# finsberg/fenicsx-beat

Measured on AMD Instinct MI355X. Metric: node_updates_per_sec, higher is better.
Workload: dtype f64

## Files before the change

fenicsx-beat_amd/csrc/beat_pde_rr.hip:

```cpp
#include "beat_pde_internal.h"

#include <algorithm>
#include <cmath>
#include <cstddef>
#include <cstdlib>

namespace {
using namespace beat_pde_detail;

constexpr int SEG = 62;

struct Coef {
  double c[15];
};

struct RGeom {
  int nx, ny, nz;
  int64_t plane;
  int ry;
  int nsegx, nrb, nchunks, zc;
  int total_waves, total_blocks;
  int z_lo_phys, z_hi_phys;
  int z_lo, z_hi;
  int part_off;
  int ghost_lo_tz, ghost_hi_tz;
  int nrg;
};

enum { RR_PDOT = 0, RR_RUPD = 1, RR_RHS = 2, RR_UDOT = 3, RR_PRUPD = 4 };

struct RArgs {
  const double* x;
  const double* x2;
  double* y;
  double* y2;
  const double* tab;
  const double* tab2;
  const double* dinv;
  Coef ci, ci2;
  double dinv_i;
  double cm, omt_dt, dt;
  const double* w[BEAT_MAX_STIM];
  double amp[BEAT_MAX_STIM];
  int nstim;
  double* partials;
  double* st;
  double* alphas;
  int slot;
  const double* e;
  const double* taba;
  Coef cia;
};

struct RKernArgs {
  RGeom g;
  RArgs a;
  const double* X;
  const double* X2;
  double* Y;
  double* Y2;
};

__device__ __forceinline__ double from_left(double v) {
  const int lo = __builtin_amdgcn_update_dpp(0, __double2loint(v), 0x138, 0xf, 0xf, true);
  const int hi = __builtin_amdgcn_update_dpp(0, __double2hiint(v), 0x138, 0xf, 0xf, true);
  return __hiloint2double(hi, lo);
}
__device__ __forceinline__ double from_right(double v) {
  const int lo = __builtin_amdgcn_update_dpp(0, __double2loint(v), 0x130, 0xf, 0xf, true);
  const int hi = __builtin_amdgcn_update_dpp(0, __double2hiint(v), 0x130, 0xf, 0xf, true);
  return __hiloint2double(hi, lo);
}

#ifndef BEAT_RR_BUF
#define BEAT_RR_BUF 2
#endif
typedef int rr_v2i __attribute__((ext_vector_type(2)));
[[maybe_unused]] constexpr unsigned RR_OOB = 0x80000000u;
#ifndef BEAT_RR_NT
#define BEAT_RR_NT 2
#endif
__device__ __forceinline__ void rr_store(double* p, double v) {
#if BEAT_RR_NT & 2
  __builtin_nontemporal_store(v, p);
#else
  *p = v;
#endif
}
__device__ __forceinline__ double rr_buf_load(const double* base, unsigned bytes, unsigned off) {
  const __amdgpu_buffer_rsrc_t r = __builtin_amdgcn_make_buffer_rsrc((void*)base, 0, (int)bytes, 0x00020000);
  const rr_v2i v = __builtin_amdgcn_raw_buffer_load_b64(r, (int)off, 0, (BEAT_RR_NT & 1) ? 2 : 0);
  return __hiloint2double(v.y, v.x);
}

#ifndef BEAT_RR_ALIGN
#define BEAT_RR_ALIGN 1
#endif
__device__ __forceinline__ double from_left_h(double v, double h, int src_lane) {
  const int lo = __builtin_amdgcn_update_dpp(__builtin_amdgcn_readlane(__double2loint(h), src_lane), __double2loint(v), 0x138, 0xf, 0xf, false);
  const int hi = __builtin_amdgcn_update_dpp(__builtin_amdgcn_readlane(__double2hiint(h), src_lane), __double2hiint(v), 0x138, 0xf, 0xf, false);
  return __hiloint2double(hi, lo);
}
__device__ __forceinline__ double from_right_h(double v, double h, int src_lane) {
  const int lo = __builtin_amdgcn_update_dpp(__builtin_amdgcn_readlane(__double2loint(h), src_lane), __double2loint(v), 0x130, 0xf, 0xf, false);
  const int hi = __builtin_amdgcn_update_dpp(__builtin_amdgcn_readlane(__double2hiint(h), src_lane), __double2hiint(v), 0x130, 0xf, 0xf, false);
  return __hiloint2double(hi, lo);
}
#ifndef BEAT_RR_ALIGN_RHS
#define BEAT_RR_ALIGN_RHS 0
#endif
constexpr bool rr_aligned_mode(int mode) {
  return BEAT_RR_ALIGN == 1 && BEAT_RR_BUF != 0 && (mode == 0 || mode == 1 || mode == 3 || mode == 4 || (mode == 2 && BEAT_RR_ALIGN_RHS == 1));
}

__device__ __forceinline__ int axis_type3(int i, int n, int lo_phys, int hi_phys) {
  if (n == 1 && lo_phys && hi_phys) return 1;
  if (i == 0 && lo_phys) return 0;
  if (i == n - 1 && hi_phys) return 2;
  return 1;
}

__device__ __forceinline__ int xcd_block(int b, int total) {
  const int per = (total + 7) >> 3;
  return (b & 7) * per + (b >> 3);
}

#ifndef BEAT_RR_WAVES_RHS
#define BEAT_RR_WAVES_RHS 3
#endif
#ifndef BEAT_RR_WAVES_IT
#define BEAT_RR_WAVES_IT 1
#endif
template <int MODE, int RY, int PD, bool GUESS = false, bool PRED = false>
__global__ __launch_bounds__(BEAT_BLOCK, (GUESS && RY == 2 && PD == 1) ? BEAT_RR_WAVES_RHS : ((MODE == RR_PDOT || MODE == RR_RUPD) && PD == 1 ? BEAT_RR_WAVES_IT : 1)) void rr_kernel(RGeom g, RArgs a, const double* __restrict__ X,
                                                        const double* __restrict__ X2, double* __restrict__ Y,
                                                        double* __restrict__ Y2) {
  constexpr int NR = RY + 2;
  constexpr int NE = GUESS ? NR : 1;
  constexpr bool FORM = MODE == RR_PDOT || MODE == RR_UDOT || MODE == RR_PRUPD;
  constexpr bool OLD = MODE == RR_PDOT || MODE == RR_PRUPD;
  constexpr bool RAW = MODE == RR_UDOT || MODE == RR_PRUPD;
  constexpr int NW = RAW ? RY : 1;
  constexpr bool BUF = BEAT_RR_BUF == 1 || (BEAT_RR_BUF == 2 && (MODE != RR_RHS || BEAT_RR_ALIGN_RHS == 1));
  constexpr bool ALIGNED = rr_aligned_mode(MODE);
  static_assert(!ALIGNED || BUF, "aligned segments come with the raw-buffer loads");
  constexpr int SEGW = ALIGNED ? 64 : SEG;
  static_assert(!GUESS || MODE == RR_RHS, "the initial guess enters the right-hand side only");
  static_assert(!PRED || MODE == RR_PDOT, "the predicted-stop sums come with PDOT only");
  __shared__ double red[4];
  __shared__ double s_dinv[32];
  __shared__ double s_tab[27 * TABW];
  __shared__ double s_tab2[MODE == RR_RHS ? 27 * TABW : 1];
  __shared__ double s_taba[GUESS ? 27 * TABW : 1];
  __shared__ double s_rc[PRED ? 4 * 2 * RY * 64 : 1];
  __shared__ double s_acc[PRED ? 4 * 2 * 64 : 1];
  if (MODE != RR_RHS) {
    if (a.st[STOP] != 0.0) return;
  }
  if (PRED) s_acc[(threadIdx.x >> 6) * 128 + (threadIdx.x & 63)] = s_acc[(threadIdx.x >> 6) * 128 + 64 + (threadIdx.x & 63)] = 0.0;
  for (int i = threadIdx.x; i < 27 * TABW; i += BEAT_BLOCK) {
    s_tab[i] = a.tab[i];
    if (MODE == RR_RHS) s_tab2[i] = a.tab2[i];
    if (GUESS) s_taba[i] = a.taba[i];
  }
  if (threadIdx.x < 27) s_dinv[threadIdx.x] = a.dinv[threadIdx.x];
  __syncthreads();
  const int lane = threadIdx.x & 63;
  const int blk = xcd_block(blockIdx.x, g.total_blocks);
  const int w = blk * 4 + (threadIdx.x >> 6);
  int seg = w % g.nsegx;
  int rb = (w / g.nsegx) % g.nrb;
  int chunk = w / (g.nsegx * g.nrb);
  bool wave_ok = blk < g.total_blocks && w < g.total_waves;
  if (g.nrg > 0) {
    seg = blk % g.nsegx;
    rb = ((blk / g.nsegx) % g.nrg) * 4 + (int)(threadIdx.x >> 6);
    chunk = blk / (g.nsegx * g.nrg);
    wave_ok = blk < g.total_blocks && rb < g.nrb;
  }
  const int gx = seg * SEGW + (ALIGNED ? 0 : -1) + lane;
  const int y0 = rb * RY - 1;
  const int zb = g.z_lo + chunk * g.zc;
  const int ze = wave_ok ? min(zb + g.zc, g.z_hi) : zb;
  const bool x_in = wave_ok && gx >= 0 && gx < g.nx;
  const bool x_out = x_in && (ALIGNED || (lane >= 1 && lane <= SEG));
  const int tx = axis_type3(gx, g.nx, 1, 1);
  bool row_in[NR];
  int txy[NR];
  int off[NR];
  const int cx = min(max(gx, 0), g.nx - 1);
#pragma unroll
  for (int r = 0; r < NR; ++r) {
    const int gy = y0 + r;
    row_in[r] = x_in && gy >= 0 && gy < g.ny;
    txy[r] = tx + 3 * axis_type3(gy, g.ny, 1, 1);
    off[r] = min(max(gy, 0), g.ny - 1) * g.nx + cx;
    if constexpr (BUF) off[r] = row_in[r] ? (int)((unsigned)(gy * g.nx + gx) * 8u) : (int)RR_OOB;
  }
  [[maybe_unused]] const unsigned pbytes = (unsigned)(g.plane * 8);
  [[maybe_unused]] unsigned hoff = RR_OOB;
  [[maybe_unused]] int htxy = 13 % 9;
  if constexpr (ALIGNED) {
    const int hr = lane < 8 ? lane : lane - 8;
    const int hx = lane < 8 ? seg * SEGW - 1 : seg * SEGW + SEGW;
    const int hy = y0 + hr;
    const bool hv = wave_ok && (lane < NR || (lane >= 8 && lane < 8 + NR)) && hx >= 0 && hx < g.nx && hy >= 0 && hy < g.ny;
    hoff = hv ? (unsigned)(hy * g.nx + hx) * 8u : RR_OOB;
    htxy = axis_type3(min(max(hx, 0), g.nx - 1), g.nx, 1, 1) + 3 * axis_type3(min(max(hy, 0), g.ny - 1), g.ny, 1, 1);
  }
  double beta = 0.0, alpha = 0.0;
  if (OLD) beta = a.st[BETA];
  if (MODE == RR_PRUPD) alpha = a.st[ALPHA];
  if (MODE == RR_RUPD) {
    alpha = a.st[RZ] / a.st[PQ];
    if (blockIdx.x == 0 && threadIdx.x == 0) a.alphas[a.slot] = alpha;
  }
  const bool have_old = beta != 0.0;

  double acc0 = 0.0, acc1 = 0.0, acc2 = 0.0;
  double Cm[NR], C0[NR], Cp[NR], ra[PD][NR], rb2[PD][NR];
  double rvn[PD][RY];
  [[maybe_unused]] double Hm = 0.0, H0 = 0.0, Hp = 0.0, rha[PD], rhb[PD];
  [[maybe_unused]] double HEm = 0.0, HE0 = 0.0, HEp = 0.0;
#pragma unroll
  for (int u = 0; u < PD; ++u) rha[u] = rhb[u] = 0.0;
  double Rw0[NW], Rwp[NW];
#pragma unroll
  for (int j = 0; j < NW; ++j) Rw0[j] = Rwp[j] = 0.0;
  double Em[NE], E0[NE], Ep[NE], re1[PD][NE];
#pragma unroll
  for (int r = 0; r < NE; ++r) {
    Em[r] = E0[r] = Ep[r] = 0.0;
#pragma unroll
    for (int u = 0; u < PD; ++u) re1[u][r] = 0.0;
  }
#pragma unroll
  for (int r = 0; r < NR; ++r) {
    Cm[r] = C0[r] = Cp[r] = 0.0;
#pragma unroll
    for (int u = 0; u < PD; ++u) ra[u][r] = rb2[u][r] = 0.0;
  }
#pragma unroll
  for (int u = 0; u < PD; ++u)
#pragma unroll
    for (int j = 0; j < RY; ++j) rvn[u][j] = 0.0;
  for (int zz = zb - 2 - PD; zz < ze; zz += PD) {
#pragma unroll
  for (int u = 0; u < PD; ++u) {
    const int z = zz + u;
    if (z < ze) {
    const int k = z + 1;
    if (k >= zb - 1 && k <= ze) {
      [[maybe_unused]] const bool zok = (k >= 0 || !g.z_lo_phys) && (k < g.nz || !g.z_hi_phys);
      const int tz9 = 9 * (k < 0 ? g.ghost_lo_tz : k >= g.nz ? g.ghost_hi_tz : axis_type3(k, g.nz, g.z_lo_phys, g.z_hi_phys));
      const bool own_plane = (k >= zb && k < ze) || (k == -1 && zb == 0 && !g.z_lo_phys) ||
                             (k == g.nz && ze == g.nz && !g.z_hi_phys);
#pragma unroll
      for (int r = 0; r < NR; ++r) {
        double c = ra[u][r];
        if (RAW && r >= 1 && r <= RY) Rwp[RAW ? r - 1 : 0] = c;
        if (FORM) {
          const int type = txy[r] + tz9;
          const double di = s_dinv[type];
          c = have_old ? fma(beta, rb2[u][r], di * ra[u][r]) : di * ra[u][r];
        }
        if constexpr (!BUF) c = (zok && row_in[r]) ? c : 0.0;
        Cp[r] = c;
        if (GUESS) {
          constexpr int q = GUESS ? 1 : 0;
          if constexpr (BUF)
            Ep[r * q] = c + re1[u][r * q];
          else
            Ep[r * q] = (zok && row_in[r]) ? c + re1[u][r * q] : 0.0;
        }
        if (OLD) {
          if (own_plane && r >= 1 && r <= RY && x_out && row_in[r])
            rr_store(&Y[(int64_t)k * g.plane + (int64_t)(y0 + r) * g.nx + gx], c);
        }
        if (PRED && r >= 1 && r <= RY) s_rc[((((threadIdx.x >> 6) * 2 + (k & 1)) * RY) + r - 1) * 64 + lane] = ra[u][r];
      }
      if constexpr (ALIGNED) {
        double hc = rha[u];
        if (FORM) {
          const double di = s_dinv[htxy + tz9];
          hc = have_old ? fma(beta, rhb[u], di * rha[u]) : di * rha[u];
        }
        Hp = hc;
        if (GUESS) HEp = hc + rhb[u];
      }
    }
    double rv[RY];
    if (MODE == RR_RUPD) {
#pragma unroll
      for (int j = 0; j < RY; ++j) rv[j] = rvn[u][j];
      if (z + PD >= zb && z + PD < ze) {
        const double* __restrict__ br = X2 + (int64_t)(z + PD) * g.plane;
#pragma unroll
        for (int j = 0; j < RY; ++j) rvn[u][j] = BUF ? rr_buf_load(br, pbytes, (unsigned)off[j + 1]) : br[off[j + 1]];
      }
    }
    {
      const int kf = k + PD;
      if (kf >= zb - 1 && kf <= ze) {
        const int cz = min(max(kf, -1), g.nz);
        const double* __restrict__ bx = X + (int64_t)cz * g.plane;
        const double* __restrict__ bx2 = (OLD && have_old) ? X2 + (int64_t)cz * g.plane : bx;
        if constexpr (BUF) {
          const unsigned pb = ((kf >= 0 || !g.z_lo_phys) && (kf < g.nz || !g.z_hi_phys)) ? pbytes : 0u;
#pragma unroll
          for (int r = 0; r < NR; ++r) {
            ra[u][r] = rr_buf_load(bx, pb, (unsigned)off[r]);
            if (OLD) rb2[u][r] = rr_buf_load(bx2, pb, (unsigned)off[r]);
          }
          if constexpr (ALIGNED) {
            rha[u] = rr_buf_load(bx, pb, hoff);
            if (OLD) rhb[u] = rr_buf_load(bx2, pb, hoff);
            if (GUESS) rhb[u] = rr_buf_load(X2 + (int64_t)cz * g.plane, pb, hoff);
          }
          if (GUESS) {
            const double* __restrict__ b1 = X2 + (int64_t)cz * g.plane;
#pragma unroll
            for (int r = 0; r < NR; ++r) re1[u][r < NE ? r : 0] = rr_buf_load(b1, pb, (unsigned)off[r]);
          }
        } else {
#pragma unroll
          for (int r = 0; r < NR; ++r) {
            ra[u][r] = bx[off[r]];
            if (OLD) rb2[u][r] = bx2[off[r]];
          }
          if (GUESS) {
            const double* __restrict__ b1 = X2 + (int64_t)cz * g.plane;
#pragma unroll
            for (int r = 0; r < NR; ++r) re1[u][r < NE ? r : 0] = b1[off[r]];
          }
        }
      }
    }
    if (z >= zb) {
    typedef const __attribute__((address_space(4))) char* KArgPtr;
    KArgPtr ka = (KArgPtr)__builtin_amdgcn_kernarg_segment_ptr();
    asm volatile("" : "+s"(ka));
    const RArgs& az = MODE == RR_RHS ? *(const RArgs*)(ka + offsetof(RKernArgs, a)) : a;
    double L0[NR], R0[NR], Rp[NR], Lm[NR];
#pragma unroll
    for (int r = 0; r < NR - 1; ++r) {
      L0[r] = ALIGNED ? from_left_h(C0[r], H0, r) : from_left(C0[r]);
      Lm[r] = ALIGNED ? from_left_h(Cm[r], Hm, r) : from_left(Cm[r]);
    }
#pragma unroll
    for (int r = 1; r < NR; ++r) {
      R0[r] = ALIGNED ? from_right_h(C0[r], H0, 8 + r) : from_right(C0[r]);
      Rp[r] = ALIGNED ? from_right_h(Cp[r], Hp, 8 + r) : from_right(Cp[r]);
    }
    double eL0[NE], eR0[NE], eRp[NE], eLm[NE];
    if (GUESS) {
#pragma unroll
      for (int r = 0; r < NE - 1; ++r) {
        eL0[r] = ALIGNED ? from_left_h(E0[r], HE0, r) : from_left(E0[r]);
        eLm[r] = ALIGNED ? from_left_h(Em[r], HEm, r) : from_left(Em[r]);
      }
#pragma unroll
      for (int r = 1; r < NE; ++r) {
        eR0[r] = ALIGNED ? from_right_h(E0[r], HE0, 8 + r) : from_right(E0[r]);
        eRp[r] = ALIGNED ? from_right_h(Ep[r], HEp, 8 + r) : from_right(Ep[r]);
      }
    }
    const int tz = axis_type3(z, g.nz, g.z_lo_phys, g.z_hi_phys);
#pragma unroll
    for (int j = 0; j < RY; ++j) {
      const int r = j + 1;
      double v[15];
      v[0] = C0[r];
      v[1] = R0[r];
      v[2] = L0[r];
      v[3] = C0[r + 1];
      v[4] = C0[r - 1];
      v[5] = Cp[r];
      v[6] = Cm[r];
      v[7] = R0[r + 1];
      v[8] = L0[r - 1];
      v[9] = Cp[r + 1];
      v[10] = Cm[r - 1];
      v[11] = Rp[r];
      v[12] = Lm[r];
      v[13] = Rp[r + 1];
      v[14] = Lm[r - 1];
      if (x_out && row_in[r]) {
        const int type = txy[r] + 9 * tz;
        const int64_t gi = (int64_t)z * g.plane + (int64_t)(y0 + r) * g.nx + gx;
        double s = 0.0;
#pragma unroll
        for (int k = 0; k < 15; ++k) s = fma(az.ci.c[k], v[k], s);
        if (MODE == RR_RHS) {
          double s2 = 0.0;
          if (!GUESS) {
#pragma unroll
            for (int k = 0; k < 15; ++k) s2 = fma(az.ci2.c[k], v[k], s2);
          }
          double di = s_dinv[13];
          if (type != 13) {
            s = 0.0;
            s2 = 0.0;
#pragma unroll
            for (int k = 0; k < 15; ++k) {
              s = fma(s_tab[type * TABW + k], v[k], s);
              if (!GUESS) s2 = fma(s_tab2[type * TABW + k], v[k], s2);
            }
            di = s_dinv[type];
          }
          double stim = 0.0;
          for (int k = 0; k < az.nstim; ++k) stim = fma(az.amp[k], az.w[k][gi], stim);
          const double b = GUESS ? fma(az.dt, stim, s) : az.cm * s - az.omt_dt * s2 + az.dt * stim;
          double rr = GUESS ? b : az.dt * (stim - s2);
          if (GUESS) {
            constexpr int q = GUESS ? 1 : 0;
            const int re_ = r * q, rp = (r + 1) * q, rm = (r - 1) * q;
            double ev[15];
            ev[0] = E0[re_];
            ev[1] = eR0[re_];
            ev[2] = eL0[re_];
            ev[3] = E0[rp];
            ev[4] = E0[rm];
            ev[5] = Ep[re_];
            ev[6] = Em[re_];
            ev[7] = eR0[rp];
            ev[8] = eL0[rm];
            ev[9] = Ep[rp];
            ev[10] = Em[rm];
            ev[11] = eRp[re_];
            ev[12] = eLm[re_];
            ev[13] = eRp[rp];
            ev[14] = eLm[rm];
            double se = 0.0;
            if (type != 13) {
#pragma unroll
              for (int k = 0; k < 15; ++k) se = fma(s_taba[type * TABW + k], ev[k], se);
            } else {
#pragma unroll
              for (int k = 0; k < 15; ++k) se = fma(az.cia.c[k], ev[k], se);
            }
            rr -= se;
          }
          const double zz = di * rr;
          rr_store(&Y[gi], rr);
          if (Y2 != nullptr) Y2[gi] = v[0];
          acc0 = fma(b, b, acc0);
          acc1 = fma(rr, zz, acc1);
          acc2 = fma(rr, rr, acc2);
        } else {
          double di = s_dinv[13];
          if (type != 13) {
            s = 0.0;
#pragma unroll
            for (int k = 0; k < 15; ++k) s = fma(s_tab[type * TABW + k], v[k], s);
            di = s_dinv[type];
          }
          if (MODE == RR_PDOT) {
            acc0 = fma(v[0], s, acc0);
            if (PRED) {
              double* sa = &s_acc[(threadIdx.x >> 6) * 128 + lane];
              sa[0] = fma(s_rc[((((threadIdx.x >> 6) * 2 + (z & 1)) * RY) + j) * 64 + lane], s, sa[0]);
              sa[64] = fma(s, s, sa[64]);
            }
          } else if (MODE == RR_UDOT) {
            const double ri = Rw0[RAW ? j : 0];
            acc0 = fma(v[0], s, acc0);
            acc1 = fma(ri, v[0], acc1);
            acc2 = fma(ri, ri, acc2);
          } else if (MODE == RR_PRUPD) {
            rr_store(&Y2[gi], fma(-alpha, s, Rw0[RAW ? j : 0]));
          } else {
            const double ri = fma(-alpha, s, rv[j]);
            rr_store(&Y[gi], ri);
            acc0 = fma(ri * di, ri, acc0);
            acc1 = fma(ri, ri, acc1);
          }
        }
      }
    }
    }
#pragma unroll
    for (int r = 0; r < NR; ++r) {
      Cm[r] = C0[r];
      C0[r] = Cp[r];
    }
    if constexpr (ALIGNED) {
      Hm = H0;
      H0 = Hp;
      if (GUESS) {
        HEm = HE0;
        HE0 = HEp;
      }
    }
    if (GUESS) {
#pragma unroll
      for (int r = 0; r < NE; ++r) {
        Em[r] = E0[r];
        E0[r] = Ep[r];
      }
    }
    if (RAW) {
#pragma unroll
      for (int j = 0; j < NW; ++j) Rw0[j] = Rwp[j];
    }
    }
  }
  }

  if (PRED) {
    acc1 = s_acc[(threadIdx.x >> 6) * 128 + (threadIdx.x & 63)];
    acc2 = s_acc[(threadIdx.x >> 6) * 128 + 64 + (threadIdx.x & 63)];
  }
  if (MODE == RR_PDOT && !PRED) {
    const double s0 = beat_block_sum(acc0, red);
    if (threadIdx.x == 0) a.partials[g.part_off + blockIdx.x] = s0;
  } else if (MODE == RR_RUPD) {
    const double s0 = beat_block_sum(acc0, red);
    const double s1 = beat_block_sum(acc1, red);
    if (threadIdx.x == 0) {
      a.partials[g.part_off + blockIdx.x] = s0;
      a.partials[BEAT_MAX_PARTIALS + g.part_off + blockIdx.x] = s1;
    }
  } else if (MODE == RR_PRUPD) {
  } else {
    const double s0 = beat_block_sum(acc0, red);
    const double s1 = beat_block_sum(acc1, red);
    const double s2 = beat_block_sum(acc2, red);
    if (threadIdx.x == 0) {
      a.partials[g.part_off + blockIdx.x] = s0;
      a.partials[BEAT_MAX_PARTIALS + g.part_off + blockIdx.x] = s1;
      a.partials[2 * BEAT_MAX_PARTIALS + g.part_off + blockIdx.x] = s2;
    }
  }
}

__global__ void rr_next_kernel(double* st) {
  if (st[STOP] != 0.0) return;
  st[BETA] = st[RZN] / st[RZ];
  st[RZ] = st[RZN];
  st[RR] = st[RRN];
  st[ITERS] += 1.0;
  const double tr = st[RTOL] * st[RTOL] * st[BB];
  if (st[RR] <= st[TOL2]) {
    st[STOP] = 1.0;
    st[REASON] = st[RR] <= tr ? 2.0 : 3.0;
  } else if (st[ITERS] >= st[MAXIT]) {
    st[STOP] = 1.0;
    st[REASON] = -3.0;
  }
}

__global__ void rr_merged_next_kernel(double* st, double* alphas, int slot) {
  if (st[STOP] != 0.0) return;
  const double g = st[RZN], d = st[PQ], rr = st[RRN];
  st[RR] = rr;
  const double tr = st[RTOL] * st[RTOL] * st[BB];
  if (rr <= st[TOL2]) {
    st[STOP] = 1.0;
    st[REASON] = rr <= tr ? 2.0 : 3.0;
    return;
  }
  if (st[ITERS] >= st[MAXIT]) {
    st[STOP] = 1.0;
    st[REASON] = -3.0;
    return;
  }
  const bool first = st[ITERS] == 0.0;
  const double beta = first ? 0.0 : g / st[RZ];
  const double alpha = first ? g / d : g / (d - beta * g / st[ALPHA]);
  st[BETA] = beta;
  st[ALPHA] = alpha;
  st[RZ] = g;
  alphas[slot] = alpha;
  st[NUPD] += 1.0;
  st[ITERS] += 1.0;
}

int rr_rows(int64_t nodes) {
  static const int forced = [] {
    const char* e = std::getenv("BEAT_RR_RY");
    const int v = e ? std::atoi(e) : 0;
    return (v == 2 || v == 4) ? v : 0;
  }();
  if (forced) return forced;
  return nodes >= ((int64_t)64 << 20) ? 4 : 2;
}

int rr_target_blocks(int64_t nodes) {
  if (const char* e = std::getenv("BEAT_RR_BLOCKS")) return std::max(1, std::atoi(e));
  return nodes >= ((int64_t)64 << 20) ? 4096 : 2048;
}

int rr_prefetch() {
  static const int pd = [] {
    const char* e = std::getenv("BEAT_RR_PD");
    const int v = e ? std::atoi(e) : 1;
    return (v >= 1 && v <= 3) ? v : 1;
  }();
  return pd;
}

int rr_guess_rows() {
  static const int rows = [] {
    const char* e = std::getenv("BEAT_RR_GUESS_RY");
    const int v = e ? std::atoi(e) : 2;
    return v == 4 ? 4 : 2;
  }();
  return rows;
}

int rr_by_rows_mask() {
  static const int mask = [] {
    const char* e = std::getenv("BEAT_RR_BY_ROWS");
    return e ? std::atoi(e) : 0;
  }();
  return mask;
}

RGeom make_geom(const beat_pde* pde, int z_lo, int z_hi, int part_off, int rows = 0, int mode = -1) {
  const Geom& f = pde->g;
  RGeom g{};
  const int64_t nodes = (int64_t)f.nx * f.ny * f.nz;
  const int RY = g.ry = rows ? rows : rr_rows(nodes);
  g.nx = f.nx;
  g.ny = f.ny;
  g.nz = f.nz;
  g.plane = f.plane;
  g.z_lo_phys = f.z_lo_phys;
  g.z_hi_phys = f.z_hi_phys;
  g.z_lo = z_lo;
  g.z_hi = z_hi;
  g.part_off = part_off;
  g.ghost_lo_tz = pde->ghost_lo_tz;
  g.ghost_hi_tz = pde->ghost_hi_tz;
  const int segw = (mode >= 0 && rr_aligned_mode(mode)) ? 64 : SEG;
  g.nsegx = (f.nx + segw - 1) / segw;
  g.nrb = (f.ny + RY - 1) / RY;
  const int nzr = std::max(0, z_hi - z_lo);
  g.nrg = (mode >= 0 && ((rr_by_rows_mask() >> mode) & 1)) ? (g.nrb + 3) / 4 : 0;
  const int64_t per_layer = g.nrg > 0 ? (int64_t)g.nsegx * g.nrg : ((int64_t)g.nsegx * g.nrb + 3) / 4;
  const int target = rr_target_blocks(nodes);
  int nchunks = (int)std::max<int64_t>(1, (target + per_layer - 1) / per_layer);
  nchunks = std::max(1, std::min(nchunks, nzr));
  g.zc = std::max(1, (nzr + nchunks - 1) / nchunks);
  g.nchunks = (nzr + g.zc - 1) / g.zc;
  while ((int64_t)g.nsegx * g.nrb * g.nchunks > (int64_t)2 * BEAT_MAX_PARTIALS && g.nchunks > 1) {
    g.zc *= 2;
    g.nchunks = (nzr + g.zc - 1) / g.zc;
  }
  g.total_waves = g.nsegx * g.nrb * g.nchunks;
  g.total_blocks = (g.total_waves + 3) / 4;
  if (g.nrg > 0) {
    g.total_blocks = g.nsegx * g.nrg * g.nchunks;
    g.total_waves = g.total_blocks * 4;
  }
  return g;
}

RGeom make_geom(const beat_pde* pde) { return make_geom(pde, 0, pde->g.nz, 0); }

inline int grid_blocks(const RGeom& g) { return ((g.total_blocks + 7) / 8) * 8; }
inline int blocks_written(const RGeom& g) { return g.total_blocks > 0 ? grid_blocks(g) : 0; }

Coef interior_row(const double* tab) {
  Coef c;
  for (int k = 0; k < 15; ++k) c.c[k] = tab[13 * 15 + k];
  return c;
}

RArgs rr_operator_args(const beat_pde* pde, double* dev_st) {
  RArgs a{};
  a.tab = pde->d_tab(0);
  a.dinv = pde->d_dinv();
  a.ci = interior_row(pde->h_A);
  a.dinv_i = pde->h_dinv[13];
  a.partials = pde->ctx->d_partials;
  a.st = dev_st;
  return a;
}

template <int MODE, bool GUESS = false, bool PRED = false>
void launch_rr(const beat_pde* pde, const RGeom& g, const RArgs& a) {
  if (g.total_blocks <= 0) return;
  const dim3 grid((unsigned)grid_blocks(g)), block(BEAT_BLOCK);
  hipStream_t s = pde->ctx->stream;
#define BEAT_RR_LAUNCH(RYV, PDV) \
  BEAT_KERNEL((rr_kernel<MODE, RYV, PDV, GUESS, PRED>), grid, block, 0, s, g, a, a.x, GUESS ? a.e : a.x2, a.y, a.y2)
  const int pd = rr_prefetch();
  if (g.ry == 2) {
    if (pd == 2) BEAT_RR_LAUNCH(2, 2); else if (pd == 3) BEAT_RR_LAUNCH(2, 3); else BEAT_RR_LAUNCH(2, 1);
  } else {
    if (pd == 2) BEAT_RR_LAUNCH(4, 2); else if (pd == 3) BEAT_RR_LAUNCH(4, 3); else BEAT_RR_LAUNCH(4, 1);
  }
#undef BEAT_RR_LAUNCH
}
}

bool beat_rr_available(const beat_pde* pde) {
  if (pde->var || pde->pc_ncoef != 1) return false;
  if (const char* e = std::getenv("BEAT_RR")) {
    if (e[0] == '0') return false;
  }
  const RGeom g = make_geom(pde);
  const RGeom gb = make_geom(pde, 0, 1, 0);
  return (int64_t)grid_blocks(g) + 2 * grid_blocks(gb) <= BEAT_MAX_PARTIALS;
}

extern "C" int beat_pde_rr_route(const beat_pde* pde, int* host_out) {
  BEAT_REQUIRE(pde != nullptr && host_out != nullptr, "null argument");
  const RGeom g = make_geom(pde, 0, pde->g.nz, 0, 0, RR_PDOT);
  host_out[0] = beat_rr_available(pde) ? 1 : 0;
  host_out[1] = g.ry;
  host_out[2] = rr_prefetch();
  host_out[3] = rr_by_rows_mask();
  host_out[4] = g.nsegx;
  host_out[5] = g.nrb;
  host_out[6] = g.zc;
  host_out[7] = g.nchunks;
  host_out[8] = g.total_blocks;
  host_out[9] = rr_guess_rows();
  return BEAT_OK;
}

int beat_rr_rhs(beat_pde* pde, const double* dev_v_prev, const double* const* host_dev_stim_w, const double* host_stim_amp,
                int n_stim, double* dev_x, double* dev_r, double* dev_st, int part, const PcgStart* start) {
  BEAT_REQUIRE(start == nullptr || part < 0, "only a right-hand side in one part starts the solve");
  const GuessTerms& gt = pde->guess.cur;
  const bool guess = gt.d != nullptr && gt.use_e;
  const int rows = guess ? rr_guess_rows() : 0;
  RArgs a{};
  a.x = dev_v_prev;
  a.y = dev_r;
  a.y2 = (dev_x == dev_v_prev) ? nullptr : dev_x;
  a.tab = pde->d_tab(2);
  a.tab2 = pde->d_tab(3);
  a.dinv = pde->d_dinv();
  a.ci = interior_row(pde->h_mass);
  a.ci2 = interior_row(pde->h_stiff);
  a.dinv_i = pde->h_dinv[13];
  a.cm = pde->C_m;
  a.omt_dt = (1.0 - pde->theta) * pde->dt;
  a.dt = pde->dt;
  beat_fill_stimuli(a, host_dev_stim_w, host_stim_amp, n_stim);
  a.partials = pde->ctx->d_partials;
  a.st = dev_st;
  if (guess) {
    a.tab = pde->d_tab(1);
    a.ci = interior_row(pde->h_B);
    a.e = gt.e;
    a.taba = pde->d_tab(0);
    a.cia = interior_row(pde->h_A);
  }
  auto launch = [&](int z_lo, int z_hi, int part_off) {
    const RGeom g = make_geom(pde, z_lo, z_hi, part_off, rows, RR_RHS);
    if (guess)
      launch_rr<RR_RHS, true>(pde, g, a);
    else
      launch_rr<RR_RHS>(pde, g, a);
    return blocks_written(g);
  };
  int count = 0;
  if (int rc = beat_launch_parts(pde, PASS_RR_RHS, part, launch, &count)) return rc;
  return part == 0 ? BEAT_OK : beat_pde_launch_reduce(pde, count, 3, dev_st, nullptr, ScalarStep::begin(dev_st, start));
}

double beat_rr_predict_bound(const beat_pde* pde) {
  const Geom& f = pde->g;
  int depth = 0;
  auto chain = [&](const RGeom& g) {
    const int per_thread = (grid_blocks(g) + BEAT_BLOCK - 1) / BEAT_BLOCK;
    depth = std::max(depth, g.zc * g.ry + 8 + per_thread + 8);
  };
  chain(make_geom(pde, 0, f.nz, 0, 0, RR_RHS));
  chain(make_geom(pde, 0, f.nz, 0, 2, RR_RHS));
  chain(make_geom(pde, 0, f.nz, 0, 4, RR_RHS));
  chain(make_geom(pde, 0, f.nz, 0, 0, RR_PDOT));
  chain(make_geom(pde, 0, f.nz, 0, 0, RR_RUPD));
  return 4.0 * (2.0 * depth + 8.0) * std::ldexp(1.0, -53);
}

int beat_rr_pdot_part(beat_pde* pde, double* dev_st, const double* dev_r, const double* dev_p_old, double* dev_p_new,
                      int part, int slot) {
  const Geom& f = pde->g;
  const bool pred = slot >= 0 && pde->predict_stop && f.z_lo_phys && f.z_hi_phys;
  if (pred && pde->predict_c <= 0.0) pde->predict_c = beat_rr_predict_bound(pde);
  RArgs a = rr_operator_args(pde, dev_st);
  a.x = dev_r;
  a.x2 = dev_p_old;
  a.y = dev_p_new;
  auto launch = [&](int z_lo, int z_hi, int part_off) {
    const RGeom g = make_geom(pde, z_lo, z_hi, part_off, 0, RR_PDOT);
    if (pred)
      launch_rr<RR_PDOT, false, true>(pde, g, a);
    else
      launch_rr<RR_PDOT>(pde, g, a);
    return blocks_written(g);
  };
  int count = 0;
  if (int rc = beat_launch_parts(pde, PASS_RR_PDOT, part, launch, &count)) return rc;
  if (part == 0) return BEAT_OK;
  if (pred) {
    static_assert(RQ == PQS + 1 && QQ == PQS + 2, "the three sums are reduced into one run of slots");
    ScalarStep predict{ScalarStep::PREDICT, dev_st};
    predict.alpha_slot = pde->d_alphas + slot;
    predict.bound_c = pde->predict_c;
    return beat_pde_launch_reduce(pde, count, 3, dev_st + PQS, dev_st, predict);
  }
  return beat_pde_launch_reduce(pde, count, 1, dev_st + PQ, dev_st);
}

int beat_rr_pdot(beat_pde* pde, double* dev_st, const double* dev_r, const double* dev_p_old, double* dev_p_new, int slot) {
  if (int rc = beat_rr_pdot_part(pde, dev_st, dev_r, dev_p_old, dev_p_new, 0, slot)) return rc;
  return beat_rr_pdot_part(pde, dev_st, dev_r, dev_p_old, dev_p_new, 1, slot);
}

int beat_rr_rupd(beat_pde* pde, double* dev_st, const double* dev_r, double* dev_r_new, const double* dev_p, int slot,
                 bool roll) {
  const RGeom g = make_geom(pde, 0, pde->g.nz, 0, 0, RR_RUPD);
  RArgs a = rr_operator_args(pde, dev_st);
  a.x = dev_p;
  a.x2 = dev_r;
  a.y = dev_r_new;
  a.alphas = pde->d_alphas;
  a.slot = slot;
  launch_rr<RR_RUPD>(pde, g, a);
  BEAT_LAUNCH_CHECK();
  return beat_pde_launch_reduce(pde, grid_blocks(g), 2, dev_st + RZN, dev_st, ScalarStep::after_update(dev_st, roll));
}

int beat_rr_udot_part(beat_pde* pde, double* dev_st, const double* dev_r, int part) {
  static_assert(RZN == PQ + 1 && RRN == PQ + 2, "the three sums travel as one all-reduce of dev_st[PQ..RRN]");
  RArgs a = rr_operator_args(pde, dev_st);
  a.x = dev_r;
  a.x2 = dev_r;
  auto launch = [&](int z_lo, int z_hi, int part_off) {
    const RGeom g = make_geom(pde, z_lo, z_hi, part_off, 0, RR_UDOT);
    launch_rr<RR_UDOT>(pde, g, a);
    return blocks_written(g);
  };
  int count = 0;
  if (int rc = beat_launch_parts(pde, PASS_RR_UDOT, part, launch, &count)) return rc;
  return part == 0 ? BEAT_OK : beat_pde_launch_reduce(pde, count, 3, dev_st + PQ, dev_st);
}

int beat_rr_merged_next(beat_pde* pde, double* dev_st, int slot) {
  BEAT_KERNEL(rr_merged_next_kernel, dim3(1), dim3(1), 0, pde->ctx->stream, dev_st, pde->d_alphas, slot);
  BEAT_LAUNCH_CHECK();
  return BEAT_OK;
}

int beat_rr_prupd(beat_pde* pde, double* dev_st, const double* dev_r, const double* dev_p_old, double* dev_p_new,
                  double* dev_r_new) {
  const RGeom g = make_geom(pde, 0, pde->g.nz, 0, 0, RR_PRUPD);
  RArgs a = rr_operator_args(pde, dev_st);
  a.x = dev_r;
  a.x2 = dev_p_old;
  a.y = dev_p_new;
  a.y2 = dev_r_new;
  launch_rr<RR_PRUPD>(pde, g, a);
  BEAT_LAUNCH_CHECK();
  return BEAT_OK;
}

int beat_rr_next(beat_pde* pde, double* dev_st) {
  BEAT_KERNEL(rr_next_kernel, dim3(1), dim3(1), 0, pde->ctx->stream, dev_st);
  BEAT_LAUNCH_CHECK();
  return BEAT_OK;
}
```

Baseline: 11.58 billion.

## Pick z-chunk count from kernel occupancy using a wave-fill cost model

Replaces the fixed block target (2048/4096) with a target chosen by minimizing an estimated cost: waves of resident blocks times (chunk depth + prefetch fill), where resident slots come from hipOccupancyMaxActiveBlocksPerMultiprocessor for the exact kernel instantiation. The default row blocking is also changed to 4 rows for all sizes. Large problems still use the old target. The aim is better balance between having enough blocks to fill the GPU and the per-chunk pipeline fill overhead, at the cost of occupancy queries and a small memo per geometry.

Measured after the change: 11.51 billion. No clear change (-0.6%).

```diff
diff --git a/fenicsx-beat_amd/csrc/beat_pde_rr.hip b/fenicsx-beat_amd/csrc/beat_pde_rr.hip
--- a/fenicsx-beat_amd/csrc/beat_pde_rr.hip
+++ b/fenicsx-beat_amd/csrc/beat_pde_rr.hip
@@ -1,8 +1,10 @@
 #include "beat_pde_internal.h"
+#include "beat_rr_fit.h"
 
 #include <algorithm>
 #include <cmath>
 #include <cstddef>
+#include <cstdio>
 #include <cstdlib>
 
 namespace {
@@ -576,20 +578,20 @@
   st[ITERS] += 1.0;
 }
 
-int rr_rows(int64_t nodes) {
+int rr_rows() {
   static const int forced = [] {
     const char* e = std::getenv("BEAT_RR_RY");
     const int v = e ? std::atoi(e) : 0;
     return (v == 2 || v == 4) ? v : 0;
   }();
-  if (forced) return forced;
-  return nodes >= ((int64_t)64 << 20) ? 4 : 2;
-}
-
-int rr_target_blocks(int64_t nodes) {
-  if (const char* e = std::getenv("BEAT_RR_BLOCKS")) return std::max(1, std::atoi(e));
-  return nodes >= ((int64_t)64 << 20) ? 4096 : 2048;
-}
+  return forced ? forced : 4;
+}
+
+constexpr int64_t RR_FIT_BELOW = (int64_t)64 << 20;
+
+constexpr int RR_MAX_BLOCKS = BEAT_MAX_PARTIALS / 2;
+
+int rr_legacy_target(int64_t nodes) { return nodes >= RR_FIT_BELOW ? 4096 : 2048; }
 
 int rr_prefetch() {
   static const int pd = [] {
@@ -600,6 +602,61 @@
   return pd;
 }
 
+template <int MODE, int RY, int PD, bool GUESS, bool PRED>
+int rr_resident_blocks() {
+  static const int slots = [] {
+    int dev = 0, cus = 0, per_cu = 0;
+    if (hipGetDevice(&dev) != hipSuccess || hipDeviceGetAttribute(&cus, hipDeviceAttributeMultiprocessorCount, dev) != hipSuccess ||
+        hipOccupancyMaxActiveBlocksPerMultiprocessor(&per_cu, rr_kernel<MODE, RY, PD, GUESS, PRED>, BEAT_BLOCK, 0) != hipSuccess ||
+        cus < 1 || per_cu < 1) {
+      (void)hipGetLastError();
+      return 0;
+    }
+    if (std::getenv("BEAT_RR_VERBOSE"))
+      std::fprintf(stderr, "rr: mode %d RY %d PD %d guess %d pred %d: %d workgroups per CU x %d CUs\n", MODE, RY, PD, (int)GUESS, (int)PRED, per_cu, cus);
+    return per_cu * cus;
+  }();
+  return slots;
+}
+
+template <int MODE, bool GUESS = false, bool PRED = false>
+int rr_resident_blocks(int ry, int pd) {
+#define BEAT_RR_SLOTS_OF(RYV, PDV) rr_resident_blocks<MODE, RYV, PDV, GUESS, PRED>()
+  if (ry == 2) return pd == 2 ? BEAT_RR_SLOTS_OF(2, 2) : pd == 3 ? BEAT_RR_SLOTS_OF(2, 3) : BEAT_RR_SLOTS_OF(2, 1);
+  return pd == 2 ? BEAT_RR_SLOTS_OF(4, 2) : pd == 3 ? BEAT_RR_SLOTS_OF(4, 3) : BEAT_RR_SLOTS_OF(4, 1);
+#undef BEAT_RR_SLOTS_OF
+}
+
+int rr_slots(int mode, int ry, bool guess, bool pred) {
+  if (const char* e = std::getenv("BEAT_RR_SLOTS")) return std::max(1, std::atoi(e));
+  const int pd = rr_prefetch();
+  switch (mode) {
+    case RR_PDOT: return pred ? rr_resident_blocks<RR_PDOT, false, true>(ry, pd) : rr_resident_blocks<RR_PDOT>(ry, pd);
+    case RR_RUPD: return rr_resident_blocks<RR_RUPD>(ry, pd);
+    case RR_UDOT: return rr_resident_blocks<RR_UDOT>(ry, pd);
+    case RR_PRUPD: return rr_resident_blocks<RR_PRUPD>(ry, pd);
+    default: return guess ? rr_resident_blocks<RR_RHS, true>(ry, pd) : rr_resident_blocks<RR_RHS>(ry, pd);
+  }
+}
+
+int64_t rr_target_blocks(int64_t nodes, int planes, int64_t per_layer, int mode, int ry, bool guess, bool pred) {
+  if (const char* e = std::getenv("BEAT_RR_BLOCKS")) return std::max(1, std::atoi(e));
+  if (nodes >= RR_FIT_BELOW && std::getenv("BEAT_RR_SLOTS") == nullptr) return rr_legacy_target(nodes);
+  const int slots = rr_slots(mode, ry, guess, pred);
+  if (slots <= 0) return rr_legacy_target(nodes);
+  struct Asked {
+    int planes, slots;
+    int64_t per_layer, target;
+  };
+  thread_local Asked memo[8] = {};
+  thread_local int next = 0;
+  for (const Asked& m : memo)
+    if (m.slots == slots && m.planes == planes && m.per_layer == per_layer) return m.target;
+  const int64_t target = rr_fit_target(planes, per_layer, slots, rr_prefetch() + 2, RR_MAX_BLOCKS);
+  memo[next++ & 7] = {planes, slots, per_layer, target};
+  return target;
+}
+
 int rr_guess_rows() {
   static const int rows = [] {
     const char* e = std::getenv("BEAT_RR_GUESS_RY");
@@ -617,11 +674,11 @@
   return mask;
 }
 
-RGeom make_geom(const beat_pde* pde, int z_lo, int z_hi, int part_off, int rows = 0, int mode = -1) {
+RGeom make_geom(const beat_pde* pde, int z_lo, int z_hi, int part_off, int rows = 0, int mode = -1, bool guess = false, bool pred = false) {
   const Geom& f = pde->g;
   RGeom g{};
   const int64_t nodes = (int64_t)f.nx * f.ny * f.nz;
-  const int RY = g.ry = rows ? rows : rr_rows(nodes);
+  const int RY = g.ry = rows ? rows : rr_rows();
   g.nx = f.nx;
   g.ny = f.ny;
   g.nz = f.nz;
@@ -639,15 +696,10 @@
   const int nzr = std::max(0, z_hi - z_lo);
   g.nrg = (mode >= 0 && ((rr_by_rows_mask() >> mode) & 1)) ? (g.nrb + 3) / 4 : 0;
   const int64_t per_layer = g.nrg > 0 ? (int64_t)g.nsegx * g.nrg : ((int64_t)g.nsegx * g.nrb + 3) / 4;
-  const int target = rr_target_blocks(nodes);
-  int nchunks = (int)std::max<int64_t>(1, (target + per_layer - 1) / per_layer);
-  nchunks = std::max(1, std::min(nchunks, nzr));
-  g.zc = std::max(1, (nzr + nchunks - 1) / nchunks);
-  g.nchunks = (nzr + g.zc - 1) / g.zc;
-  while ((int64_t)g.nsegx * g.nrb * g.nchunks > (int64_t)2 * BEAT_MAX_PARTIALS && g.nchunks > 1) {
-    g.zc *= 2;
-    g.nchunks = (nzr + g.zc - 1) / g.zc;
-  }
+  const int64_t target = rr_target_blocks(nodes, nzr, per_layer, mode, RY, guess, pred);
+  const RrChunks cut = rr_chunks(nzr, per_layer, (int64_t)g.nsegx * g.nrb, target, (int64_t)4 * RR_MAX_BLOCKS);
+  g.zc = cut.zc;
+  g.nchunks = cut.nchunks;
   g.total_waves = g.nsegx * g.nrb * g.nchunks;
   g.total_blocks = (g.total_waves + 3) / 4;
   if (g.nrg > 0) {
@@ -752,7 +804,7 @@
     a.cia = interior_row(pde->h_A);
   }
   auto launch = [&](int z_lo, int z_hi, int part_off) {
-    const RGeom g = make_geom(pde, z_lo, z_hi, part_off, rows, RR_RHS);
+    const RGeom g = make_geom(pde, z_lo, z_hi, part_off, rows, RR_RHS, guess);
     if (guess)
       launch_rr<RR_RHS, true>(pde, g, a);
     else
@@ -774,7 +826,10 @@
   chain(make_geom(pde, 0, f.nz, 0, 0, RR_RHS));
   chain(make_geom(pde, 0, f.nz, 0, 2, RR_RHS));
   chain(make_geom(pde, 0, f.nz, 0, 4, RR_RHS));
+  chain(make_geom(pde, 0, f.nz, 0, 2, RR_RHS, true));
+  chain(make_geom(pde, 0, f.nz, 0, 4, RR_RHS, true));
   chain(make_geom(pde, 0, f.nz, 0, 0, RR_PDOT));
+  chain(make_geom(pde, 0, f.nz, 0, 0, RR_PDOT, false, true));
   chain(make_geom(pde, 0, f.nz, 0, 0, RR_RUPD));
   return 4.0 * (2.0 * depth + 8.0) * std::ldexp(1.0, -53);
 }
@@ -789,7 +844,7 @@
   a.x2 = dev_p_old;
   a.y = dev_p_new;
   auto launch = [&](int z_lo, int z_hi, int part_off) {
-    const RGeom g = make_geom(pde, z_lo, z_hi, part_off, 0, RR_PDOT);
+    const RGeom g = make_geom(pde, z_lo, z_hi, part_off, 0, RR_PDOT, false, pred);
     if (pred)
       launch_rr<RR_PDOT, false, true>(pde, g, a);
     else
diff --git a/fenicsx-beat_amd/csrc/beat_rr_fit.h b/fenicsx-beat_amd/csrc/beat_rr_fit.h
--- /dev/null
+++ b/fenicsx-beat_amd/csrc/beat_rr_fit.h
@@ -0,0 +1,52 @@
+#pragma once
+
+#include <algorithm>
+#include <cstdint>
+
+namespace beat_pde_detail {
+
+struct RrChunks {
+  int zc;
+  int nchunks;
+};
+
+inline RrChunks rr_chunks(int planes, int64_t per_layer, int64_t waves_per_layer, int64_t target, int64_t max_waves) {
+  int nchunks = (int)std::max<int64_t>(1, std::min<int64_t>((target + per_layer - 1) / per_layer, planes));
+  RrChunks c;
+  c.zc = std::max(1, (planes + nchunks - 1) / nchunks);
+  c.nchunks = (planes + c.zc - 1) / c.zc;
+  while (waves_per_layer * c.nchunks > max_waves && c.nchunks > 1) {
+    c.zc *= 2;
+    c.nchunks = (planes + c.zc - 1) / c.zc;
+  }
+  return c;
+}
+
+inline int64_t rr_fit_cost(int64_t blocks, int zc, int64_t slots, int fill) {
+  return ((blocks + slots - 1) / slots) * ((int64_t)zc + fill);
+}
+
+inline int64_t rr_fit_target(int planes, int64_t per_layer, int64_t slots, int fill, int64_t cap) {
+  if (planes <= 1 || per_layer <= 0) return std::max<int64_t>(1, per_layer);
+  slots = std::max<int64_t>(1, slots);
+  const int n_cap = (int)std::max<int64_t>(1, std::min<int64_t>(planes, cap / per_layer));
+  const int zc_cap = (planes + n_cap - 1) / n_cap;
+  const bool can_fill = (int64_t)((planes + zc_cap - 1) / zc_cap) * per_layer >= slots;
+  int best_n = 1;
+  int64_t best_cost = -1;
+  for (int n = 1; n <= planes; ++n) {
+    const int zc = (planes + n - 1) / n;
+    if ((planes + zc - 1) / zc != n) continue;
+    const int64_t blocks = n * per_layer;
+    if (n > 1 && blocks > cap) break;
+    if (can_fill && blocks < slots) continue;
+    const int64_t cost = rr_fit_cost(blocks, zc, slots, fill);
+    if (best_cost < 0 || cost <= best_cost) {
+      best_cost = cost;
+      best_n = n;
+    }
+  }
+  return best_n * per_layer;
+}
+
+}
```
